# RobotLocomotion/pytorch-dense-correspondence

Measured on AMD Instinct MI355X. Metric: training images/sec, 640x480 D=3 ResNet34-8s, higher is better.
Workload: dtype f32 (f16x3 products)

## Files before the change

### pytorch-dense-correspondence_amd/csrc/dcn_common.h

```cpp
#pragma once
#include <hip/hip_runtime.h>
#include <stdint.h>

#include "dcn_hip.h"

#ifndef DCN_WAIT_VMCNT
#define DCN_WAIT_VMCNT(n) asm volatile("s_waitcnt vmcnt(" #n ")" ::: "memory")
#define DCN_WAIT_LGKMCNT0() asm volatile("s_waitcnt lgkmcnt(0)" ::: "memory")
#define DCN_OPAQUE_INT(v) asm volatile("" : "+v"(v))
#endif

#if defined(DCN_HOSTEMU_BUILD)
#define DCN_MAX_VGPRS(n)
#else
#define DCN_MAX_VGPRS(n) __attribute__((amdgpu_num_vgpr(n)))
#endif

#define DCN_SCHED_FENCE() do { asm volatile("" ::: "memory"); __builtin_amdgcn_sched_barrier(0); } while (0)

namespace dcn {

constexpr int kWave = 64;

template <class T> __device__ __forceinline__ T wave_sum(T v) {
#pragma unroll
    for (int off = kWave / 2; off > 0; off >>= 1) v += __shfl_down(v, off, kWave);
    return v;
}

template <int NT, class T> __device__ __forceinline__ T block_sum(T v, T* scratch) {
    v = wave_sum(v);
    const int lane = threadIdx.x & (kWave - 1), wv = threadIdx.x / kWave;
    __syncthreads();
    if (lane == 0) scratch[wv] = v;
    __syncthreads();
    T r = scratch[0];
    if (threadIdx.x == 0) {
#pragma unroll
        for (int i = 1; i < NT / kWave; ++i) r += scratch[i];
    }
    return r;
}

static __global__ void __launch_bounds__(256) fill_words_kernel(unsigned* __restrict__ p, unsigned v, size_t words) {
    for (size_t i = (size_t)blockIdx.x * 256 + threadIdx.x; i < words; i += (size_t)gridDim.x * 256) p[i] = v;
}
inline int fill_bytes_async(void* p, int byte_value, size_t n, hipStream_t st) {
    if (n == 0) return DCN_OK;
    if (n % 4) return DCN_E_INVALID;
    const unsigned b = (unsigned)byte_value & 0xffu, v = b | (b << 8) | (b << 16) | (b << 24);
    const size_t words = n / 4;
    size_t blocks = (words + 255) / 256;
    if (blocks > 4096) blocks = 4096;
    hipLaunchKernelGGL(fill_words_kernel, dim3((unsigned)blocks), dim3(256), 0, st, (unsigned*)p, v, words);
    return hipGetLastError() == hipSuccess ? DCN_OK : DCN_E_LAUNCH;
}

inline int check_launch() { return hipGetLastError() == hipSuccess ? DCN_OK : DCN_E_LAUNCH; }

__host__ __device__ inline int64_t ceil_div64(int64_t a, int64_t b) { return (a + b - 1) / b; }
__host__ __device__ inline int ceil_div(int a, int b) { return (a + b - 1) / b; }

}
```

### pytorch-dense-correspondence_amd/csrc/dcn_tuning.h

```cpp
#pragma once

namespace dcn {

struct Tuning {
    int conv_mode = -1;
    int conv_mode_invalid = 0;
    int backward_overlap = 1;
    int gemm_tile_m = 0;
    int gemm_sk = -1;
    double gemm_sk_min_gain = 20.0;
    int gemm_uni = 1;
    int stem8 = 1;
    int gemm_sk_inline = 1;
    int bn_bwd_fused = 0;
    int defer_residual_add = 1;
    int wgrad_splits = 0;
    int wgrad_tile = 0;
    int wgrad_deep = 4;
    int gemm_hl = 1;
    int hl_min_k = 128;
    int gemm_hl_rows = 0;
    int gemm_hlx = 1;
    int gemm_hlx_kg = 0;
    int gemm_hlx_splits = 0;
    int gemm_hlx_narrow = 1;
    double hlx_cost1 = 1.32, hlx_cost2 = 1.42, hlx_split_cost = 14.0;
    int hl_setprio = 1;
    int hlx_stagger = 1;
    int hlx_counters = 1;
    int wgrad_hl_min_m = 0;
    int wgrad_hl = 1;
    int wgrad_hlr = 1;
    int wgrad_hlr_min_m = 0;
    int wgrad_hlr_pairs = 1;
    int hl_producers = 1;
    int hl_only_mid = 1;
    int stem_pool_fused = 1;
    int bn_reduce_wide = 32;
    int wsplit_overlap = 1;
    int bn_nt = 0;
    int bn_reverse = 0;
    int bn_bwd_lean = 1;
    int bn_bwd_lean_mask = 7;
    int wgrad_roles = 1;
};

const Tuning& tuning();

}
```

### pytorch-dense-correspondence_amd/csrc/dcn_tuning.hip

```cpp
#include <atomic>
#include <cstdio>
#include <cstdlib>
#include <cstring>
#include <mutex>

#include "dcn_common.h"
#include "dcn_tuning.h"

namespace dcn {
namespace {

Tuning g_tuning;
std::once_flag g_once;
std::mutex g_mu;

void read_env(Tuning& t) {
    t = Tuning();
    if (const char* m = getenv("DCN_CONV_MODE")) {
        if (!strcmp(m, "fp32")) t.conv_mode = DCN_CONV_FP32;
        else if (!strcmp(m, "f16x3")) t.conv_mode = DCN_CONV_F16X3;
        else t.conv_mode_invalid = 1;
    }
    if (const char* e = getenv("DCN_BACKWARD_OVERLAP")) t.backward_overlap = atoi(e) != 0;
    if (const char* e = getenv("DCN_GEMM_TILE_M")) t.gemm_tile_m = atoi(e);
    if (const char* e = getenv("DCN_GEMM_SK")) t.gemm_sk = atoi(e);
    if (const char* e = getenv("DCN_GEMM_SK_MIN_GAIN")) t.gemm_sk_min_gain = atof(e);
    if (const char* e = getenv("DCN_STEM8")) t.stem8 = atoi(e) != 0;
    if (const char* e = getenv("DCN_GEMM_UNI")) t.gemm_uni = atoi(e) != 0;
    if (const char* e = getenv("DCN_GEMM_SK_FIXUP")) t.gemm_sk_inline = strcmp(e, "kernel") != 0;
    if (const char* e = getenv("DCN_BN_BWD_FUSED")) t.bn_bwd_fused = atoi(e) != 0;
    if (const char* e = getenv("DCN_DEFER_RESIDUAL_ADD")) t.defer_residual_add = atoi(e) != 0;
    if (const char* e = getenv("DCN_WGRAD_DEEP")) t.wgrad_deep = atoi(e);
    if (const char* e = getenv("DCN_WGRAD_ROLES")) t.wgrad_roles = atoi(e);
    if (const char* e = getenv("DCN_WGRAD_TILE")) t.wgrad_tile = atoi(e);
    if (const char* e = getenv("DCN_WGRAD_SPLITS")) t.wgrad_splits = atoi(e);
    if (const char* e = getenv("DCN_GEMM_HL")) t.gemm_hl = atoi(e);
    if (const char* e = getenv("DCN_GEMM_HL_ROWS")) t.gemm_hl_rows = atoi(e);
    if (const char* e = getenv("DCN_HL_MIN_K")) { const int v = atoi(e); if (v >= 32) t.hl_min_k = v; }
    if (const char* e = getenv("DCN_GEMM_HLX")) {
        int a = 0, b = 0;
        if (strchr(e, ',')) {
            if (sscanf(e, "%d,%d", &a, &b) == 2) {
                t.gemm_hlx = 1;
                t.gemm_hlx_kg = (a == 1 || a == 2) ? a : 0;
                t.gemm_hlx_splits = b > 0 ? b : 0;
            }
        } else {
            t.gemm_hlx = atoi(e) != 0;
        }
    }
    if (const char* e = getenv("DCN_GEMM_HLX_NARROW")) t.gemm_hlx_narrow = atoi(e) != 0;
    if (const char* e = getenv("DCN_HLX_COST")) {
        double a = 0, b = 0, c = 0;
        if (sscanf(e, "%lf,%lf,%lf", &a, &b, &c) == 3 && a > 0 && b > 0 && c >= 0) { t.hlx_cost1 = a; t.hlx_cost2 = b; t.hlx_split_cost = c; }
    }
    if (const char* e = getenv("DCN_HL_ONLY_MID")) t.hl_only_mid = atoi(e);
    if (const char* e = getenv("DCN_STEM_POOL_FUSED")) t.stem_pool_fused = atoi(e);
    if (const char* e = getenv("DCN_WGRAD_HL")) t.wgrad_hl = atoi(e);
    if (const char* e = getenv("DCN_HL_SETPRIO")) t.hl_setprio = atoi(e) != 0;
    if (const char* e = getenv("DCN_HLX_STAGGER")) { const int v = atoi(e); t.hlx_stagger = (v >= 0 && v <= 2) ? v : 1; }
    if (const char* e = getenv("DCN_HLX_COUNTERS")) t.hlx_counters = atoi(e) != 0;
    if (const char* e = getenv("DCN_WGRAD_HL_MIN_M")) t.wgrad_hl_min_m = atoi(e);
    if (const char* e = getenv("DCN_WGRAD_HLR")) t.wgrad_hlr = atoi(e);
    if (const char* e = getenv("DCN_WGRAD_HLR_MIN_M")) t.wgrad_hlr_min_m = atoi(e);
    if (const char* e = getenv("DCN_WGRAD_HLR_PAIRS")) t.wgrad_hlr_pairs = atoi(e);
    if (const char* e = getenv("DCN_HL_PRODUCERS")) t.hl_producers = atoi(e) != 0;
    if (const char* e = getenv("DCN_BN_REVERSE")) t.bn_reverse = atoi(e);
    if (const char* e = getenv("DCN_BN_NT")) t.bn_nt = atoi(e);
    if (const char* e = getenv("DCN_WSPLIT_OVERLAP")) t.wsplit_overlap = atoi(e) != 0;
    if (const char* e = getenv("DCN_BN_REDUCE_WIDE")) t.bn_reduce_wide = atoi(e);
    if (const char* e = getenv("DCN_BN_BWD_LEAN")) t.bn_bwd_lean = atoi(e) != 0;
    if (const char* e = getenv("DCN_BN_BWD_LEAN_MASK")) t.bn_bwd_lean_mask = atoi(e) & 7;
}

}

const Tuning& tuning() {
    std::call_once(g_once, [] { read_env(g_tuning); });
    return g_tuning;
}

}

extern "C" void dcn_reload_env(void) {
    (void)dcn::tuning();
    std::lock_guard<std::mutex> lock(dcn::g_mu);
    dcn::read_env(dcn::g_tuning);
}
```

### pytorch-dense-correspondence_amd/csrc/elementwise_kernels.hip

```cpp
#include "dcn_tuning.h"
#include "elementwise_kernels.h"
#include "f16_split.h"

namespace dcn {

__device__ __forceinline__ void wave_atomic_absmax(float amax, float* absmax) {
#pragma unroll
    for (int o = 32; o > 0; o >>= 1) amax = fmaxf(amax, __shfl_xor(amax, o));
    if ((threadIdx.x & 63) == 0 && amax > 0.f) {
        const unsigned bits = __float_as_uint(amax);
        if (bits > __atomic_load_n(reinterpret_cast<unsigned*>(absmax), __ATOMIC_RELAXED))
            atomicMax(reinterpret_cast<unsigned*>(absmax), bits);
    }
}

__global__ void __launch_bounds__(256)
nchw3_to_nhwc4_kernel(const float* __restrict__ img, float* __restrict__ out, int hw, int64_t total,
                      float* __restrict__ absmax) {
    __shared__ float s_m[4];
    float m = 0.f;
    for (int64_t i = (int64_t)blockIdx.x * 256 + threadIdx.x; i < total; i += (int64_t)gridDim.x * 256) {
        const int64_t n = i / hw, p = i - n * hw;
        const float* s = img + n * 3 * hw + p;
        const float4 v = make_float4(s[0], s[hw], s[2 * (int64_t)hw], 0.f);
// ... 411 lines not shown
        dgamma[c] = (float)tot_b;
    }
    if (absmax && threadIdx.x < 64) {
        bound = fmaxf(bound, __shfl_xor(bound, 1));
        bound = fmaxf(bound, __shfl_xor(bound, 2));
        if (threadIdx.x == 0) {
            const unsigned bits = __float_as_uint(bound);
            const unsigned seen = LEAN ? __atomic_load_n(reinterpret_cast<unsigned*>(absmax), __ATOMIC_RELAXED) : pre_bound;
            if (bound > 0.f && bits > seen)
                atomicMax(reinterpret_cast<unsigned*>(absmax), bits);
        }
    }
}
#define DCN_BN_FIN_ARGS const float* __restrict__ partial, int chunks, int groups, int C, double count,                        \
                        const float* __restrict__ gamma, const float* __restrict__ invstd, int gstride,                        \
                        float* __restrict__ dgamma, float* __restrict__ dbeta, float* __restrict__ k123, float* __restrict__ absmax
#define DCN_BN_FIN_PASS partial, chunks, groups, C, count, gamma, invstd, gstride, dgamma, dbeta, k123, absmax
__global__ void __launch_bounds__(256)
bn_bwd_finalize_kernel(DCN_BN_FIN_ARGS) { bn_bwd_finalize_body<false>(DCN_BN_FIN_PASS); }
__global__ void __launch_bounds__(256) DCN_MAX_VGPRS(48)
bn_bwd_finalize_lean_kernel(DCN_BN_FIN_ARGS) { bn_bwd_finalize_body<true>(DCN_BN_FIN_PASS); }
#undef DCN_BN_FIN_ARGS
#undef DCN_BN_FIN_PASS

__global__ void __launch_bounds__(256)
bn_bwd_apply_kernel(const float* __restrict__ dy, const float* dy2, const float* __restrict__ relu_out,
                    const unsigned char* __restrict__ relu_mask, const float* __restrict__ x,
                    const float* __restrict__ mean, const float* __restrict__ invstd, const float* __restrict__ k1,
                    const float* __restrict__ k2, const float* __restrict__ k3, float* __restrict__ dx,
                    float* g_out, int c4n, int64_t total4, int64_t group4, int gstride, int kstride, int rev) {
    for (int64_t j = (int64_t)blockIdx.x * 256 + threadIdx.x; j < total4; j += (int64_t)gridDim.x * 256) {
        const int64_t i = rev ? total4 - 1 - j : j;
        const int c0 = (int)(i % c4n) * 4;
        const bool second = i >= group4;
        const int c = c0 + (second ? gstride : 0), ck = c0 + (second ? kstride : 0);
        const float4 g = relu_masked(load_dy(dy, dy2, i), relu_out, relu_mask, i);
        const float4 v = reinterpret_cast<const float4*>(x)[i];
        const float4 mu = *reinterpret_cast<const float4*>(mean + c);
        const float4 is = *reinterpret_cast<const float4*>(invstd + c);
        const float4 a = *reinterpret_cast<const float4*>(k1 + ck);
        const float4 b = *reinterpret_cast<const float4*>(k2 + ck);
        const float4 d = *reinterpret_cast<const float4*>(k3 + ck);
        float4 o;
        o.x = a.x * (g.x - b.x - (v.x - mu.x) * is.x * d.x);
        o.y = a.y * (g.y - b.y - (v.y - mu.y) * is.y * d.y);
        o.z = a.z * (g.z - b.z - (v.z - mu.z) * is.z * d.z);
        o.w = a.w * (g.w - b.w - (v.w - mu.w) * is.w * d.w);
        reinterpret_cast<float4*>(dx)[i] = o;
        if (g_out) reinterpret_cast<float4*>(g_out)[i] = g;
    }
}

template <bool LEAN, bool DQ>
__device__ __forceinline__ void
bn_bwd_apply_blocked_body(const float* __restrict__ dy, const float* dy2, const float* __restrict__ relu_out,
                          const unsigned char* __restrict__ relu_mask, const float* __restrict__ x,
                          const float* __restrict__ mean, const float* __restrict__ invstd, const float* __restrict__ k1,
                          const float* __restrict__ k2, const float* __restrict__ k3, float* __restrict__ dx,
                          float* g_out, dcnsplit::u32x4* __restrict__ dq, const float* __restrict__ absmax,
                          int c4n, int64_t rows, int64_t rows_per_group, int gstride, int kstride,
                          dcnsplit::u32x2* __restrict__ hl, int rev, int nt) {
    const float s = dcnsplit::pow2_scale(*absmax);
    const int64_t total = ((rows + 3) >> 2) * c4n;
    for (int64_t j = (int64_t)blockIdx.x * 256 + threadIdx.x; j < total; j += (int64_t)gridDim.x * 256) {
        const int64_t i = rev ? total - 1 - j : j;
        const int64_t q = i / c4n;
        const int cq = (int)(i - q * c4n);
        const bool second = q * 4 >= rows_per_group;
        int c = cq * 4 + (second ? gstride : 0), ck = cq * 4 + (second ? kstride : 0);
        float4 mu, is, a, b, d;
        if (!LEAN) {
            mu = *reinterpret_cast<const float4*>(mean + c);
            is = *reinterpret_cast<const float4*>(invstd + c);
            a = *reinterpret_cast<const float4*>(k1 + ck);
            b = *reinterpret_cast<const float4*>(k2 + ck);
            d = *reinterpret_cast<const float4*>(k3 + ck);
        }
        float o[4][4];
#pragma unroll
        for (int r = 0; r < 4; ++r) {
            const int64_t m = q * 4 + r;
            if (LEAN) __builtin_amdgcn_sched_barrier(0);
            if (m < rows) {
                const int64_t e = m * c4n + cq;

                float4 g0 = ld4(dy, e, nt != 0);
                if (dy2) {
                    const float4 h = reinterpret_cast<const float4*>(dy2)[e];
                    g0.x += h.x; g0.y += h.y; g0.z += h.z; g0.w += h.w;
                }
                float4 g = relu_masked(g0, relu_out, relu_mask, e);
                float4 v = ld4(x, e, nt != 0);
                if (LEAN) {
                    DCN_OPAQUE_INT(g.x); DCN_OPAQUE_INT(g.y); DCN_OPAQUE_INT(g.z); DCN_OPAQUE_INT(g.w);
                    DCN_OPAQUE_INT(v.x); DCN_OPAQUE_INT(v.y); DCN_OPAQUE_INT(v.z); DCN_OPAQUE_INT(v.w);
                    DCN_OPAQUE_INT(c); DCN_OPAQUE_INT(ck);
                }
                if (LEAN && DQ) {
#define DCN_BN_STEP(dst, expr, ptr)                                                                                           \
                    { const float4 k = *reinterpret_cast<const float4*>(ptr);                                                  \
                      dst = expr;                                                                                              \
                      DCN_OPAQUE_INT(dst.x); DCN_OPAQUE_INT(dst.y); DCN_OPAQUE_INT(dst.z); DCN_OPAQUE_INT(dst.w); }
                    float4 t, u;
                    DCN_BN_STEP(t, make_float4(v.x - k.x, v.y - k.y, v.z - k.z, v.w - k.w), mean + c)
                    DCN_BN_STEP(t, make_float4(t.x * k.x, t.y * k.y, t.z * k.z, t.w * k.w), invstd + c)
                    DCN_BN_STEP(t, make_float4(t.x * k.x, t.y * k.y, t.z * k.z, t.w * k.w), k3 + ck)
                    DCN_BN_STEP(u, make_float4(g.x - k.x, g.y - k.y, g.z - k.z, g.w - k.w), k2 + ck)
                    DCN_BN_STEP(t, make_float4(k.x * (u.x - t.x), k.y * (u.y - t.y), k.z * (u.z - t.z), k.w * (u.w - t.w)), k1 + ck)
#undef DCN_BN_STEP
                    o[r][0] = t.x; o[r][1] = t.y; o[r][2] = t.z; o[r][3] = t.w;
                } else {
                    if (LEAN) {
                        mu = *reinterpret_cast<const float4*>(mean + c);
                        is = *reinterpret_cast<const float4*>(invstd + c);
                        a = *reinterpret_cast<const float4*>(k1 + ck);
                        b = *reinterpret_cast<const float4*>(k2 + ck);
                        d = *reinterpret_cast<const float4*>(k3 + ck);
                    }
                    o[r][0] = a.x * (g.x - b.x - (v.x - mu.x) * is.x * d.x);
                    o[r][1] = a.y * (g.y - b.y - (v.y - mu.y) * is.y * d.y);
                    o[r][2] = a.z * (g.z - b.z - (v.z - mu.z) * is.z * d.z);
                    o[r][3] = a.w * (g.w - b.w - (v.w - mu.w) * is.w * d.w);
                }
                if (dx) reinterpret_cast<float4*>(dx)[e] = make_float4(o[r][0], o[r][1], o[r][2], o[r][3]);
                if (g_out) reinterpret_cast<float4*>(g_out)[e] = g;
                if (hl) {
                    dcnsplit::h4 ha, hb;
                    dcnsplit::split4(make_float4(o[r][0], o[r][1], o[r][2], o[r][3]), s, ha, hb);
                    dcnsplit::u32x2* line = hl + (e >> 3) * 16 + (e & 7);
                    line[0] = __builtin_bit_cast(dcnsplit::u32x2, ha);
                    line[8] = __builtin_bit_cast(dcnsplit::u32x2, hb);
                }
            } else {
                o[r][0] = o[r][1] = o[r][2] = o[r][3] = 0.f;
            }
        }
        if (DQ && dq) dcnsplit::store_blocked_quad(dq, q, cq, c4n, o, s);
    }
}
#define DCN_BN_APB_ARGS const float* __restrict__ dy, const float* dy2, const float* __restrict__ relu_out,                    \
                        const unsigned char* __restrict__ relu_mask, const float* __restrict__ x,                              \
                        const float* __restrict__ mean, const float* __restrict__ invstd, const float* __restrict__ k1,        \
                        const float* __restrict__ k2, const float* __restrict__ k3, float* __restrict__ dx,                    \
                        float* g_out, dcnsplit::u32x4* __restrict__ dq, const float* __restrict__ absmax,                      \
                        int c4n, int64_t rows, int64_t rows_per_group, int gstride, int kstride,                               \
                        dcnsplit::u32x2* __restrict__ hl, int rev, int nt
#define DCN_BN_APB_PASS dy, dy2, relu_out, relu_mask, x, mean, invstd, k1, k2, k3, dx, g_out, dq, absmax, c4n, rows, rows_per_group, \
                        gstride, kstride, hl, rev, nt
__global__ void __launch_bounds__(256)
bn_bwd_apply_blocked_kernel(DCN_BN_APB_ARGS) { bn_bwd_apply_blocked_body<false, true>(DCN_BN_APB_PASS); }
template <bool DQ>
__global__ void __launch_bounds__(256) DCN_MAX_VGPRS(48)
bn_bwd_apply_blocked_lean_kernel(DCN_BN_APB_ARGS) { bn_bwd_apply_blocked_body<true, DQ>(DCN_BN_APB_PASS); }
#undef DCN_BN_APB_ARGS
#undef DCN_BN_APB_PASS

__global__ void __launch_bounds__(256)
absmax_kernel(const float* __restrict__ v, int64_t total, float* __restrict__ absmax) {
    float amax = 0.f;
    for (int64_t i = (int64_t)blockIdx.x * 256 + threadIdx.x; i < total; i += (int64_t)gridDim.x * 256)
        amax = fmaxf(amax, fabsf(v[i]));
    wave_atomic_absmax(amax, absmax);
}

__global__ void __launch_bounds__(256)
add_kernel(const float* __restrict__ a, const float* __restrict__ b, float* __restrict__ out, int64_t total4) {
    for (int64_t i = (int64_t)blockIdx.x * 256 + threadIdx.x; i < total4; i += (int64_t)gridDim.x * 256) {
        const float4 u = reinterpret_cast<const float4*>(a)[i], v = reinterpret_cast<const float4*>(b)[i];
        reinterpret_cast<float4*>(out)[i] = make_float4(u.x + v.x, u.y + v.y, u.z + v.z, u.w + v.w);
    }
}

__global__ void __launch_bounds__(256)
maxpool_fwd_kernel(const float* __restrict__ in, float* __restrict__ out, unsigned char* __restrict__ argmax, int hin,
                   int win, int hout, int wout, int c4n, int64_t total4, const float* __restrict__ scale,
                   const float* __restrict__ shift, int gstride, int64_t group_n, unsigned char* __restrict__ relu_mask) {
    const int64_t i = (int64_t)blockIdx.x * 256 + threadIdx.x;
    if (i >= total4) return;
    const int c4 = (int)(i % c4n);
    int64_t pix = i / c4n;
    const int ox = (int)(pix % wout); pix /= wout;
    const int oy = (int)(pix % hout);
    const int64_t n = pix / hout;
    float4 sc = make_float4(1.f, 1.f, 1.f, 1.f), sh = make_float4(0.f, 0.f, 0.f, 0.f);
    if (scale) {
        const int c = c4 * 4 + (n >= group_n ? gstride : 0);
        sc = *reinterpret_cast<const float4*>(scale + c);
        sh = *reinterpret_cast<const float4*>(shift + c);
    }
    float4 best = make_float4(-INFINITY, -INFINITY, -INFINITY, -INFINITY);
    int bx = -1, by = -1, bz = -1, bw = -1;
    for (int r = 0; r < 3; ++r) {
        const int iy = oy * 2 - 1 + r;
        if (iy < 0 || iy >= hin) continue;
        for (int s = 0; s < 3; ++s) {
            const int ix = ox * 2 - 1 + s;
            if (ix < 0 || ix >= win) continue;
            const int64_t src = ((n * hin + iy) * win + ix) * c4n + c4;
            float4 v = reinterpret_cast<const float4*>(in)[src];
            if (scale) {
                v = make_float4(v.x * sc.x + sh.x, v.y * sc.y + sh.y, v.z * sc.z + sh.z, v.w * sc.w + sh.w);
                v.x = fmaxf(v.x, 0.f); v.y = fmaxf(v.y, 0.f); v.z = fmaxf(v.z, 0.f); v.w = fmaxf(v.w, 0.f);
                if (relu_mask)
                    relu_mask[src] = (unsigned char)((v.x > 0.f ? 1 : 0) | (v.y > 0.f ? 2 : 0) | (v.z > 0.f ? 4 : 0) | (v.w > 0.f ? 8 : 0));
            }
            const int t = r * 3 + s;
            if (v.x > best.x || bx < 0 || v.x != v.x) { best.x = v.x; bx = t; }
            if (v.y > best.y || by < 0 || v.y != v.y) { best.y = v.y; by = t; }
            if (v.z > best.z || bz < 0 || v.z != v.z) { best.z = v.z; bz = t; }
            if (v.w > best.w || bw < 0 || v.w != v.w) { best.w = v.w; bw = t; }
        }
    }
    reinterpret_cast<float4*>(out)[i] = best;
    if (argmax) {
        unsigned char* a = argmax + i * 4;
        a[0] = (unsigned char)bx; a[1] = (unsigned char)by; a[2] = (unsigned char)bz; a[3] = (unsigned char)bw;
    }
}

__global__ void __launch_bounds__(256)
maxpool_bwd_kernel(const float* __restrict__ gout, const float* __restrict__ gout2, const unsigned char* __restrict__ argmax,
                   float* __restrict__ gin, int hin, int win, int hout, int wout, int c4n, int64_t total4) {
    const int64_t i = (int64_t)blockIdx.x * 256 + threadIdx.x;
    if (i >= total4) return;
    const int c4 = (int)(i % c4n);
    int64_t pix = i / c4n;
    const int ix = (int)(pix % win); pix /= win;
    const int iy = (int)(pix % hin);
    const int64_t n = pix / hin;
    float4 acc = make_float4(0.f, 0.f, 0.f, 0.f);
    for (int oy = iy / 2; oy <= (iy + 1) / 2; ++oy) {
        if (oy >= hout) continue;
        const int r = iy - (oy * 2 - 1);
        if (r < 0 || r > 2) continue;
        for (int ox = ix / 2; ox <= (ix + 1) / 2; ++ox) {
            if (ox >= wout) continue;
            const int s = ix - (ox * 2 - 1);
            if (s < 0 || s > 2) continue;
            const int t = r * 3 + s;
            const int64_t o = ((n * hout + oy) * wout + ox) * c4n + c4;
            float4 g = reinterpret_cast<const float4*>(gout)[o];
            if (gout2) {
                const float4 h = reinterpret_cast<const float4*>(gout2)[o];
                g.x += h.x; g.y += h.y; g.z += h.z; g.w += h.w;
            }
            const unsigned char* a = argmax + o * 4;
            if (a[0] == t) acc.x += g.x;
            if (a[1] == t) acc.y += g.y;
            if (a[2] == t) acc.z += g.z;
            if (a[3] == t) acc.w += g.w;
        }
    }
    reinterpret_cast<float4*>(gin)[i] = acc;
}

__device__ __forceinline__ void src_index(int dst, float scale, int in_size, int& i0, int& i1, float& l1) {
    const float s = scale * (float)dst;
    i0 = (int)s;
    if (i0 > in_size - 1) i0 = in_size - 1;
    i1 = i0 < in_size - 1 ? i0 + 1 : i0;
    l1 = s - (float)i0;
}

__global__ void __launch_bounds__(256)
upsample_fwd_kernel(const float* __restrict__ low, int hl, int wl, int ldl, int d, int h, int w, float sh, float sw,
                    int normalize, float* __restrict__ out, int64_t total) {
    const int64_t i = (int64_t)blockIdx.x * 256 + threadIdx.x;
    if (i >= total) return;
    const int x = (int)(i % w);
    const int64_t t = i / w;
    const int y = (int)(t % h);
    const int64_t n = t / h;
    int y0, y1, x0, x1;
    float ly, lx;
    src_index(y, sh, hl, y0, y1, ly);
    src_index(x, sw, wl, x0, x1, lx);
    const float hy = 1.f - ly, hx = 1.f - lx;
    const float* p00 = low + ((n * hl + y0) * wl + x0) * ldl;
    const float* p01 = low + ((n * hl + y0) * wl + x1) * ldl;
    const float* p10 = low + ((n * hl + y1) * wl + x0) * ldl;
    const float* p11 = low + ((n * hl + y1) * wl + x1) * ldl;
    float* o = out + i * d;
    if (!normalize) {
        for (int k = 0; k < d; ++k) o[k] = hy * (hx * p00[k] + lx * p01[k]) + ly * (hx * p10[k] + lx * p11[k]);
    } else {
        float ss = 0.f;
        for (int k = 0; k < d; ++k) {
            const float v = hy * (hx * p00[k] + lx * p01[k]) + ly * (hx * p10[k] + lx * p11[k]);
            ss = fmaf(v, v, ss);
        }
        const float nrm = sqrtf(ss);
        for (int k = 0; k < d; ++k)
            o[k] = (hy * (hx * p00[k] + lx * p01[k]) + ly * (hx * p10[k] + lx * p11[k])) / nrm;
    }
}

__global__ void __launch_bounds__(256)
normalize_bwd_kernel(const float* __restrict__ low, int hl, int wl, int ldl, int d, int h, int w, float sh, float sw,
                     const float* __restrict__ gout, float* __restrict__ gv, int64_t total) {
    const int64_t i = (int64_t)blockIdx.x * 256 + threadIdx.x;
    if (i >= total) return;
    const int x = (int)(i % w);
    const int64_t t = i / w;
    const int y = (int)(t % h);
    const int64_t n = t / h;
    int y0, y1, x0, x1;
    float ly, lx;
    src_index(y, sh, hl, y0, y1, ly);
    src_index(x, sw, wl, x0, x1, lx);
    const float hy = 1.f - ly, hx = 1.f - lx;
    const float* p00 = low + ((n * hl + y0) * wl + x0) * ldl;
    const float* p01 = low + ((n * hl + y0) * wl + x1) * ldl;
    const float* p10 = low + ((n * hl + y1) * wl + x0) * ldl;
    const float* p11 = low + ((n * hl + y1) * wl + x1) * ldl;
    const float* g = gout + i * d;
    float ss = 0.f, dot = 0.f;
    for (int k = 0; k < d; ++k) {
        const float v = hy * (hx * p00[k] + lx * p01[k]) + ly * (hx * p10[k] + lx * p11[k]);
        ss = fmaf(v, v, ss);
        dot = fmaf(v, g[k], dot);
    }
    const float nrm = sqrtf(ss), inv = 1.f / nrm;
    dot *= inv;
    for (int k = 0; k < d; ++k) {
        const float v = hy * (hx * p00[k] + lx * p01[k]) + ly * (hx * p10[k] + lx * p11[k]);
        gv[i * d + k] = (g[k] - v * inv * dot) * inv;
    }
}

__global__ void __launch_bounds__(256)
upsample_bwd_rows_kernel(const float* __restrict__ gout, int hl, int d, int h, int w, float sh, float* __restrict__ tmp,
                         int64_t total) {
    const int64_t i = (int64_t)blockIdx.x * 256 + threadIdx.x;
    if (i >= total) return;
    const int64_t wd = (int64_t)w * d;
    const int64_t xd = i % wd;
    const int64_t t = i / wd;
    const int iy = (int)(t % hl);
    const int64_t n = t / hl;
    const float inv = sh > 0.f ? 1.f / sh : 0.f;
    int ylo = (int)floorf(((float)iy - 1.f) * inv) - 1, yhi = (int)ceilf(((float)iy + 1.f) * inv) + 1;
    if (ylo < 0) ylo = 0;
    if (yhi > h - 1 || sh <= 0.f) yhi = h - 1;
    float acc = 0.f;
    for (int y = ylo; y <= yhi; ++y) {
        int y0, y1;
        float ly;
        src_index(y, sh, hl, y0, y1, ly);
        float wgt = 0.f;
        if (y0 == iy) wgt += 1.f - ly;
        if (y1 == iy) wgt += ly;
        if (wgt != 0.f) acc = fmaf(wgt, gout[(n * h + y) * wd + xd], acc);
    }
    tmp[i] = acc;
}
__global__ void __launch_bounds__(256)
upsample_bwd_cols_kernel(const float* __restrict__ tmp, int hl, int wl, int ldl, int d, int w, float sw,
                         float* __restrict__ glow, int64_t total) {
    const int64_t i = (int64_t)blockIdx.x * 256 + threadIdx.x;
    if (i >= total) return;
    const int k = (int)(i % ldl);
    const int64_t t = i / ldl;
    const int ix = (int)(t % wl);
    const int64_t row = t / wl;
    if (k >= d) { glow[i] = 0.f; return; }
    const float inv = sw > 0.f ? 1.f / sw : 0.f;
    int xlo = (int)floorf(((float)ix - 1.f) * inv) - 1, xhi = (int)ceilf(((float)ix + 1.f) * inv) + 1;
    if (xlo < 0) xlo = 0;
    if (xhi > w - 1 || sw <= 0.f) xhi = w - 1;
    float acc = 0.f;
    for (int x = xlo; x <= xhi; ++x) {
        int x0, x1;
        float lx;
        src_index(x, sw, wl, x0, x1, lx);
        float wgt = 0.f;
        if (x0 == ix) wgt += 1.f - lx;
        if (x1 == ix) wgt += lx;
        if (wgt != 0.f) acc = fmaf(wgt, tmp[(row * w + x) * d + k], acc);
    }
    glow[i] = acc;
}

static inline unsigned blocks_for(int64_t n, int cap = 0) {
    int64_t b = ceil_div64(n, 256);
    if (cap > 0 && b > cap) b = cap;
    if (b < 1) b = 1;
    return (unsigned)b;
}
constexpr int kGridCap = 256 * 8;

thread_local const LaunchObserver* launch_observer = nullptr;

void launch_nchw3_to_nhwc4(const float* img, float* out, int n, int hw, float* absmax, hipStream_t st) {
    const int64_t total = (int64_t)n * hw;
    ObservedLaunch obs(DCN_PROF_RESAMPLE, 28.0 * (double)total, st);
    hipLaunchKernelGGL(nchw3_to_nhwc4_kernel, dim3(blocks_for(total, kGridCap)), dim3(256), 0, st, img, out, hw, total, absmax);
}
void launch_pad_c3_to_c4(const float* w, float* wp, int64_t rows, hipStream_t st) {
    ObservedLaunch obs(DCN_PROF_OTHER, 28.0 * (double)rows, st);
    hipLaunchKernelGGL(pad_c3_to_c4_kernel, dim3(blocks_for(rows)), dim3(256), 0, st, w, wp, rows);
}
void launch_unpad_c4_to_c3(const float* wp, float* w, int64_t rows, hipStream_t st) {
    ObservedLaunch obs(DCN_PROF_OTHER, 28.0 * (double)rows, st);
    hipLaunchKernelGGL(unpad_c4_to_c3_kernel, dim3(blocks_for(rows)), dim3(256), 0, st, wp, w, rows);
}
void launch_pad_rows(const float* src, float* dst, int64_t rows, int d, int ld, hipStream_t st) {
    ObservedLaunch obs(DCN_PROF_OTHER, 4.0 * (double)rows * (d + ld), st);
    hipLaunchKernelGGL(pad_rows_kernel, dim3(blocks_for(rows * ld)), dim3(256), 0, st, src, dst, rows, d, ld);
}
void launch_bn_finalize(const float* partial, int tiles_per_group, int groups, int C, double count_per_group,
                        const float* gamma, const float* beta, float* rmean, float* rvar, float momentum, float eps,
                        int training, float* stats, float* out_bound, const float* res_bound, hipStream_t st) {
    ObservedLaunch obs(DCN_PROF_BN_FINALIZE, training ? 12.0 * (double)tiles_per_group * groups * C : 0.0, st);
    hipLaunchKernelGGL(bn_finalize_kernel, dim3(ceil_div(C, 4)), dim3(256), 0, st, partial, tiles_per_group, groups, C,
                       count_per_group, gamma, beta, rmean, rvar, momentum, eps, training, stats, stats + C, stats + 2 * C,
                       stats + 3 * C, 4 * C, out_bound, res_bound);
}
void launch_bn_apply(const float* x, const float* stats1, const float* res, const float* stats2, int relu, float* y,
                     unsigned char* relu_mask, int C, int64_t rows, int groups, hipStream_t st, void* hl_out,
                     const float* hl_absmax) {
    const int64_t total4 = rows * (C / 4);
    if ((C % 32) != 0 || !hl_absmax) hl_out = nullptr;
    ObservedLaunch obs(DCN_PROF_BN_APPLY, (double)rows * C * (4.0 + (res ? 4.0 : 0.0) + (y ? 4.0 : 0.0) + (hl_out ? 4.0 : 0.0) +
                                                             (relu_mask ? 0.25 : 0.0)), st);
    hipLaunchKernelGGL(bn_apply_kernel, dim3(blocks_for(total4, kGridCap)), dim3(256), 0, st, x, stats1, stats1 + C, res,
                       stats2, stats2 ? stats2 + C : nullptr, relu, y, relu_mask, C / 4, total4, total4 / groups, 4 * C,
                       (dcnsplit::u32x2*)hl_out, hl_absmax, tuning().bn_reverse & 1, tuning().bn_nt & 1);
}
int bn_bwd_chunks(int64_t rows_per_group) {
    const int rows = rows_per_group >= 16384 ? 128 : (rows_per_group >= 8192 ? 64 : 32);
    int64_t chunks = ceil_div64(rows_per_group, rows);
    if (chunks > 1024) chunks = 1024;
    if (chunks < 1) chunks = 1;
    return (int)chunks;
}
void launch_bn_bwd(const float* dy, const float* relu_out, const unsigned char* relu_mask, const float* x, const float* stats,
                   const float* gamma, int C,
                   int64_t rows, int groups, float* partial, float* dgamma, float* dbeta, float* k123, float* dx,
                   float* g_out, float* absmax, void* dq, hipStream_t st, int reduced_tiles_per_group, const float* dy2,
                   void* hl_dx, int keep_dx, int lean) {
    const int64_t rpg = rows / groups;
    const float* mean = stats + 2 * C;
    const float* invstd = stats + 3 * C;
    int chunks = reduced_tiles_per_group;
    const double in_bytes = 8.0 + (dy2 ? 4.0 : 0.0) + (relu_mask ? 0.25 : (relu_out ? 4.0 : 0.0));
    if (chunks <= 0) {
        chunks = bn_bwd_chunks(rpg);
        const int rpc = (int)ceil_div64(rpg, chunks);
        ObservedLaunch obs(DCN_PROF_BN_BWD_REDUCE, (double)rows * C * in_bytes, st);
        const int cap = tuning().bn_reduce_wide;
        const int cq = ((C % 512) == 0 && cap >= 128) ? 128 : (((C % 256) == 0 && cap >= 64) ? 64 : (((C % 128) == 0 && cap >= 32) ? 32 : 16));
#define DCN_BN_RED(K, CQ)                                                                                                     \
        hipLaunchKernelGGL(K<CQ>, dim3(ceil_div(C, 4 * CQ), chunks * groups), dim3(256), 0, st, dy, dy2, relu_out,            \
                           relu_mask, x, mean, invstd, C, rpg, chunks, 4 * C, rpc, partial)
#define DCN_BN_RED_CQ(K)                                                                                                      \
        if (cq == 128) DCN_BN_RED(K, 128);                                                                                    \
        else if (cq == 64) DCN_BN_RED(K, 64);                                                                                 \
        else if (cq == 32) DCN_BN_RED(K, 32);                                                                                 \
        else DCN_BN_RED(K, 16)
        if (lean & 1) { DCN_BN_RED_CQ(bn_bwd_reduce_lean_kernel); }
        else { DCN_BN_RED_CQ(bn_bwd_reduce_kernel); }
#undef DCN_BN_RED_CQ
#undef DCN_BN_RED
    }
    {
        ObservedLaunch obs(DCN_PROF_BN_FINALIZE, 16.0 * (double)chunks * groups * C, st);
        const auto kernel = (lean & 2) ? bn_bwd_finalize_lean_kernel : bn_bwd_finalize_kernel;
        hipLaunchKernelGGL(kernel, dim3(ceil_div(C, 4)), dim3(256), 0, st,
                           (const float*)partial, chunks, groups, C, (double)rpg, gamma, invstd, 4 * C, dgamma, dbeta, k123, absmax);
    }
    const int64_t total4 = rows * (C / 4);
    if ((dq || (hl_dx && (C % 32) == 0)) && absmax) {
        const bool hl = hl_dx && (C % 32) == 0;
        ObservedLaunch obs(DCN_PROF_BN_BWD_APPLY, (double)rows * C * (in_bytes + ((hl && !keep_dx) ? 0.0 : 4.0) + (g_out ? 4.0 : 0.0) +
                                                                      (dq ? 4.0 : 0.0) + (hl ? 4.0 : 0.0)), st);
        const auto kernel = !(lean & 4) ? bn_bwd_apply_blocked_kernel
                                        : (dq ? bn_bwd_apply_blocked_lean_kernel<true> : bn_bwd_apply_blocked_lean_kernel<false>);
        hipLaunchKernelGGL(kernel, dim3(blocks_for(((rows + 3) / 4) * (C / 4), kGridCap)), dim3(256), 0, st,
                           dy, dy2, relu_out, relu_mask, x, mean, invstd, (const float*)k123, (const float*)(k123 + C),
                           (const float*)(k123 + 2 * C), (hl_dx && (C % 32) == 0 && !keep_dx) ? nullptr : dx, g_out,
                           (dcnsplit::u32x4*)dq, (const float*)absmax, C / 4, rows, rpg, 4 * C, 3 * C,
                           (C % 32) == 0 ? (dcnsplit::u32x2*)hl_dx : nullptr, (tuning().bn_reverse >> 1) & 1, (tuning().bn_nt >> 1) & 1);
        return;
    }
    ObservedLaunch obs(DCN_PROF_BN_BWD_APPLY, (double)rows * C * (in_bytes + 4.0 + (g_out ? 4.0 : 0.0)), st);
    hipLaunchKernelGGL(bn_bwd_apply_kernel, dim3(blocks_for(total4, kGridCap)), dim3(256), 0, st, dy, dy2, relu_out, relu_mask,
                       x, mean, invstd, (const float*)k123, (const float*)(k123 + C), (const float*)(k123 + 2 * C), dx, g_out,
                       C / 4, total4, total4 / groups, 4 * C, 3 * C, (tuning().bn_reverse >> 1) & 1);
}
void launch_add(const float* a, const float* b, float* out, int64_t n, hipStream_t st) {
    ObservedLaunch obs(DCN_PROF_OTHER, 12.0 * (double)n, st);
    hipLaunchKernelGGL(add_kernel, dim3(blocks_for(n / 4, kGridCap)), dim3(256), 0, st, a, b, out, n / 4);
}
void launch_maxpool_fwd(const float* in, float* out, unsigned char* argmax, int n, int hin, int win, int hout,
                        int wout, int C, hipStream_t st, const float* bn_stats, int groups, unsigned char* relu_mask) {
    const int64_t total4 = (int64_t)n * hout * wout * (C / 4);
    ObservedLaunch obs(DCN_PROF_RESAMPLE, (double)n * C * ((double)hin * win * (4.0 + (bn_stats && relu_mask ? 0.25 : 0.0)) +
                                                          (double)hout * wout * (4.0 + (argmax ? 1.0 : 0.0))), st);
    hipLaunchKernelGGL(maxpool_fwd_kernel, dim3(blocks_for(total4)), dim3(256), 0, st, in, out, argmax, hin, win, hout,
                       wout, C / 4, total4, bn_stats, bn_stats ? bn_stats + C : nullptr, 4 * C,
                       (int64_t)(groups > 1 ? n / groups : n), bn_stats ? relu_mask : nullptr);
}
void launch_maxpool_bwd(const float* gout, const unsigned char* argmax, float* gin, int n, int hin, int win, int hout,
                        int wout, int C, hipStream_t st, const float* gout2) {
    const int64_t total4 = (int64_t)n * hin * win * (C / 4);
    ObservedLaunch obs(DCN_PROF_RESAMPLE, (double)n * C * ((double)hin * win * 4.0 + (double)hout * wout * (5.0 + (gout2 ? 4.0 : 0.0))), st);
    hipLaunchKernelGGL(maxpool_bwd_kernel, dim3(blocks_for(total4)), dim3(256), 0, st, gout, gout2, argmax, gin, hin, win,
                       hout, wout, C / 4, total4);
}
static inline float ac_scale(int in, int out) { return out > 1 ? (float)(in - 1) / (float)(out - 1) : 0.f; }
void launch_upsample_fwd(const float* low, int n, int hl, int wl, int ldl, int d, int h, int w, int normalize,
                         float* out, hipStream_t st) {
    const int64_t total = (int64_t)n * h * w;
    ObservedLaunch obs(DCN_PROF_RESAMPLE, 4.0 * ((double)n * hl * wl * ldl + (double)total * d), st);
    hipLaunchKernelGGL(upsample_fwd_kernel, dim3(blocks_for(total)), dim3(256), 0, st, low, hl, wl, ldl, d, h, w,
                       ac_scale(hl, h), ac_scale(wl, w), normalize, out, total);
}
size_t upsample_bwd_tmp_bytes(int n, int hl, int w, int d) { return (size_t)n * hl * w * d * sizeof(float); }
void launch_normalize_bwd(const float* low, int n, int hl, int wl, int ldl, int d, int h, int w, const float* gout,
                          float* gv, hipStream_t st) {
    const int64_t total = (int64_t)n * h * w;
    ObservedLaunch obs(DCN_PROF_RESAMPLE, 4.0 * ((double)n * hl * wl * ldl + 2.0 * (double)total * d), st);
    hipLaunchKernelGGL(normalize_bwd_kernel, dim3(blocks_for(total)), dim3(256), 0, st, low, hl, wl, ldl, d, h, w,
                       ac_scale(hl, h), ac_scale(wl, w), gout, gv, total);
}
void launch_upsample_bwd(const float* gout, int n, int hl, int wl, int ldl, int d, int h, int w, float* tmp,
                         float* glow, float* absmax, hipStream_t st, const float* gout_b) {
    const int64_t t1 = (int64_t)n * hl * w * d;
    if (gout_b) {
        const int64_t th = t1 / 2;
        for (int k = 0; k < 2; ++k) {
            ObservedLaunch obs(DCN_PROF_RESAMPLE, 4.0 * ((double)(n / 2) * h * w * d + (double)th), st);
            hipLaunchKernelGGL(upsample_bwd_rows_kernel, dim3(blocks_for(th)), dim3(256), 0, st, k ? gout_b : gout, hl, d, h, w,
                               ac_scale(hl, h), tmp + k * th, th);
        }
    } else {
        ObservedLaunch obs(DCN_PROF_RESAMPLE, 4.0 * ((double)n * h * w * d + (double)t1), st);
        hipLaunchKernelGGL(upsample_bwd_rows_kernel, dim3(blocks_for(t1)), dim3(256), 0, st, gout, hl, d, h, w,
                           ac_scale(hl, h), tmp, t1);
    }
    const int64_t t2 = (int64_t)n * hl * wl * ldl;
    {
        ObservedLaunch obs(DCN_PROF_RESAMPLE, 4.0 * ((double)t1 + (double)t2), st);
        hipLaunchKernelGGL(upsample_bwd_cols_kernel, dim3(blocks_for(t2)), dim3(256), 0, st, (const float*)tmp, hl, wl, ldl,
                           d, w, ac_scale(wl, w), glow, t2);
    }
    if (absmax) {
        ObservedLaunch obs(DCN_PROF_OTHER, 4.0 * (double)t2, st);
        hipLaunchKernelGGL(absmax_kernel, dim3(blocks_for(t2, 256)), dim3(256), 0, st, (const float*)glow, t2, absmax);
    }
}

}

extern "C" int dcn_upsample_forward(const float* low, int n, int hl, int wl, int ldl, int d, int h, int w, int normalize,
                                    float* out, void* stream) {
    if (!low || !out || n < 1 || hl < 1 || wl < 1 || d < 1 || ldl < d || h < 1 || w < 1) return DCN_E_INVALID;
    dcn::launch_upsample_fwd(low, n, hl, wl, ldl, d, h, w, normalize, out, (hipStream_t)stream);
    return dcn::check_launch();
}

extern "C" size_t dcn_upsample_backward_tmp_bytes(int n, int hl, int w, int d) {
    return dcn::upsample_bwd_tmp_bytes(n, hl, w, d);
}

extern "C" int dcn_upsample_backward(const float* gout, int n, int hl, int wl, int ldl, int d, int h, int w, float* glow,
                                     float* tmp, void* stream) {
    if (!gout || !glow || !tmp || n < 1 || hl < 1 || wl < 1 || d < 1 || ldl < d || h < 1 || w < 1) return DCN_E_INVALID;
    dcn::launch_upsample_bwd(gout, n, hl, wl, ldl, d, h, w, tmp, glow, nullptr, (hipStream_t)stream);
    return dcn::check_launch();
}

extern "C" int dcn_bn_forward(const float* x, const float* bn_partial, int mtiles, int c, int64_t rows, const float* gamma,
                              const float* beta, float* running_mean, float* running_var, float momentum, float eps,
                              int training, const float* res, int relu, float* y, unsigned char* relu_mask, float* stats,
                              void* stream) {
    if (!x || !gamma || !beta || !y || !stats || c < 4 || (c % 4) != 0 || rows < 1) return DCN_E_INVALID;
    if (training ? (!bn_partial || mtiles < 1) : (!running_mean || !running_var)) return DCN_E_INVALID;
    hipStream_t st = (hipStream_t)stream;
    dcn::launch_bn_finalize(bn_partial, mtiles, 1, c, (double)rows, gamma, beta, running_mean, running_var, momentum, eps,
                            training, stats, nullptr, nullptr, st);
    dcn::launch_bn_apply(x, stats, res, nullptr, relu, y, relu_mask, c, rows, 1, st);
    return dcn::check_launch();
}

extern "C" size_t dcn_bn_backward_workspace(int64_t rows, int c) {
    if (rows < 1 || c < 4) return 0;
    return ((size_t)dcn::bn_bwd_chunks(rows) * 4 * (size_t)c + 3 * (size_t)c) * sizeof(float);
}

extern "C" int dcn_bn_backward(const float* dy, const unsigned char* relu_mask, const float* x, const float* stats,
                               const float* gamma, int c, int64_t rows, float* dgamma, float* dbeta, float* dx, float* g_out,
                               void* workspace, void* stream) {
    if (!dy || !x || !stats || !gamma || !dgamma || !dbeta || !dx || !workspace || c < 4 || (c % 4) != 0 || rows < 1)
        return DCN_E_INVALID;
    float* partial = (float*)workspace;
    float* k123 = partial + (size_t)dcn::bn_bwd_chunks(rows) * 4 * c;
    dcn::launch_bn_bwd(dy, nullptr, relu_mask, x, stats, gamma, c, rows, 1, partial, dgamma, dbeta, k123, dx, g_out, nullptr,
                       nullptr, (hipStream_t)stream, 0, nullptr, nullptr, 0, dcn::tuning().bn_bwd_lean ? dcn::tuning().bn_bwd_lean_mask : 0);
    return dcn::check_launch();
}

extern "C" int dcn_bn_backward_from_partial(const float* dy, const float* bn_partial, int mtiles, const float* x,
                                            const float* stats, const float* gamma, int c, int64_t rows, float* dgamma,
                                            float* dbeta, float* dx, void* workspace, void* stream) {
    if (!dy || !bn_partial || mtiles < 1 || !x || !stats || !gamma || !dgamma || !dbeta || !dx || !workspace || c < 4 ||
        (c % 4) != 0 || rows < 1)
        return DCN_E_INVALID;
    dcn::launch_bn_bwd(dy, nullptr, nullptr, x, stats, gamma, c, rows, 1, const_cast<float*>(bn_partial), dgamma, dbeta,
                       (float*)workspace, dx, nullptr, nullptr, nullptr, (hipStream_t)stream, mtiles, nullptr, nullptr, 0,
                       dcn::tuning().bn_bwd_lean ? dcn::tuning().bn_bwd_lean_mask : 0);
    return dcn::check_launch();
}

extern "C" size_t dcn_bn_backward_full_workspace(int64_t rows, int c, int groups) {
    if (rows < 1 || c < 4 || groups < 1 || (rows % groups) != 0) return 0;
    return ((size_t)groups * dcn::bn_bwd_chunks(rows / groups) * 4 * (size_t)c + (size_t)groups * 3 * (size_t)c) * sizeof(float);
}

extern "C" int dcn_bn_backward_full(const float* dy, const float* dy2, const float* relu_out, const unsigned char* relu_mask,
                                    const float* x, const float* stats, const float* gamma, int c, int64_t rows, int groups,
                                    float* dgamma, float* dbeta, float* dx, float* g_out, float* absmax, void* dq, void* hl_dx,
                                    int keep_dx, void* workspace, void* stream) {
    if (!dy || !x || !stats || !gamma || !dgamma || !dbeta || !workspace || c < 4 || (c % 4) != 0 || rows < 1) return DCN_E_INVALID;
    if ((groups != 1 && groups != 2) || (rows % groups) != 0) return DCN_E_INVALID;
    const bool blocked = (dq || (hl_dx && (c % 32) == 0)) && absmax;
    if ((dq || hl_dx) && !absmax) return DCN_E_INVALID;
    if (hl_dx && (c % 32) != 0) return DCN_E_INVALID;
    if (blocked && groups == 2 && ((rows / groups) % 4) != 0) return DCN_E_INVALID;
    if (!dx && !(hl_dx && !keep_dx)) return DCN_E_INVALID;
// ... 21 lines not shown
```

Baseline: 470.0.

## Add software-pipelined deep BN backward apply kernel with LDS-staged coefficients

Adds a new blocked BN backward apply kernel that issues loads for several rows ahead (depth 2 or 3) before computing, so memory latency overlaps with arithmetic. Per-channel mean, invstd and k coefficients are staged once per block in shared memory instead of being reloaded per element. Specialised template variants remove runtime branches for the mask, dy2, dx, g_out and hl outputs. It is selected by default for C<=512 and up to two groups. The cost is more register pressure under a 48-VGPR cap and more code variants.

Result: faster. 481.7 (median of 6 runs) (+2.5%).

```diff
diff --git a/pytorch-dense-correspondence_amd/csrc/dcn_common.h b/pytorch-dense-correspondence_amd/csrc/dcn_common.h
--- a/pytorch-dense-correspondence_amd/csrc/dcn_common.h
+++ b/pytorch-dense-correspondence_amd/csrc/dcn_common.h
@@ -14,6 +14,12 @@
 #define DCN_MAX_VGPRS(n)
 #else
 #define DCN_MAX_VGPRS(n) __attribute__((amdgpu_num_vgpr(n)))
+#endif
+
+#if defined(DCN_HOSTEMU_BUILD)
+#define DCN_OPAQUE_UNIFORM(v) ((void)(v))
+#else
+#define DCN_OPAQUE_UNIFORM(v) asm volatile("" : "+s"(v))
 #endif
 
 #define DCN_SCHED_FENCE() do { asm volatile("" ::: "memory"); __builtin_amdgcn_sched_barrier(0); } while (0)
diff --git a/pytorch-dense-correspondence_amd/csrc/dcn_tuning.h b/pytorch-dense-correspondence_amd/csrc/dcn_tuning.h
--- a/pytorch-dense-correspondence_amd/csrc/dcn_tuning.h
+++ b/pytorch-dense-correspondence_amd/csrc/dcn_tuning.h
@@ -42,6 +42,7 @@
     int bn_reverse = 0;
     int bn_bwd_lean = 1;
     int bn_bwd_lean_mask = 7;
+    int bn_bwd_lean_depth = 3;
     int wgrad_roles = 1;
 };
 
diff --git a/pytorch-dense-correspondence_amd/csrc/dcn_tuning.hip b/pytorch-dense-correspondence_amd/csrc/dcn_tuning.hip
--- a/pytorch-dense-correspondence_amd/csrc/dcn_tuning.hip
+++ b/pytorch-dense-correspondence_amd/csrc/dcn_tuning.hip
@@ -71,6 +71,7 @@
     if (const char* e = getenv("DCN_BN_REDUCE_WIDE")) t.bn_reduce_wide = atoi(e);
     if (const char* e = getenv("DCN_BN_BWD_LEAN")) t.bn_bwd_lean = atoi(e) != 0;
     if (const char* e = getenv("DCN_BN_BWD_LEAN_MASK")) t.bn_bwd_lean_mask = atoi(e) & 7;
+    if (const char* e = getenv("DCN_BN_BWD_LEAN_DEPTH")) { const int v = atoi(e); t.bn_bwd_lean_depth = v < 1 ? 1 : (v > 3 ? 3 : v); }
 }
 
 }
diff --git a/pytorch-dense-correspondence_amd/csrc/elementwise_kernels.hip b/pytorch-dense-correspondence_amd/csrc/elementwise_kernels.hip
--- a/pytorch-dense-correspondence_amd/csrc/elementwise_kernels.hip
+++ b/pytorch-dense-correspondence_amd/csrc/elementwise_kernels.hip
@@ -587,6 +587,145 @@
 template <bool DQ>
 __global__ void __launch_bounds__(256) DCN_MAX_VGPRS(48)
 bn_bwd_apply_blocked_lean_kernel(DCN_BN_APB_ARGS) { bn_bwd_apply_blocked_body<true, DQ>(DCN_BN_APB_PASS); }
+
+struct BnBwdRow { float4 g, h, v; unsigned m; };
+__device__ __forceinline__ const float* bn_at(const float* p, unsigned bytes) {
+    return reinterpret_cast<const float*>(reinterpret_cast<const char*>(p) + bytes);
+}
+template <bool DY2, bool MASK>
+__device__ __forceinline__ void bn_bwd_row_issue(BnBwdRow& w, const float* x_b, const float* dy_b, const float* dy2_b,
+                                                 const unsigned char* mask_b, unsigned o) {
+    w.v = *reinterpret_cast<const float4*>(bn_at(x_b, 16u * o));
+    w.g = *reinterpret_cast<const float4*>(bn_at(dy_b, 16u * o));
+    if (DY2) w.h = *reinterpret_cast<const float4*>(bn_at(dy2_b, 16u * o));
+    if (MASK) w.m = mask_b[o];
+}
+template <bool DY2, bool MASK>
+__device__ __forceinline__ float4 bn_bwd_row_grad(const BnBwdRow& w) {
+    float4 g = w.g;
+    if (DY2) { g.x += w.h.x; g.y += w.h.y; g.z += w.h.z; g.w += w.h.w; }
+    if (MASK) {
+        const unsigned m = w.m;
+        g.x = (m & 1u) ? g.x : 0.f; g.y = (m & 2u) ? g.y : 0.f; g.z = (m & 4u) ? g.z : 0.f; g.w = (m & 8u) ? g.w : 0.f;
+    }
+    return g;
+}
+#define DCN_OPAQUE_F4(v) do { DCN_OPAQUE_INT(v.x); DCN_OPAQUE_INT(v.y); DCN_OPAQUE_INT(v.z); DCN_OPAQUE_INT(v.w); } while (0)
+constexpr int kBnDeepPitch = 2 * 128;
+template <int D, bool DQ, bool DY2, bool MASK, int GOUT, int DX, int HL, bool GUARD>
+__device__ __forceinline__ void
+bn_bwd_apply_deep_body(int64_t j0, const float* __restrict__ dy, const float* dy2, const unsigned char* __restrict__ relu_mask,
+                       const float* __restrict__ x, float* __restrict__ dx, float* g_out, dcnsplit::u32x4* __restrict__ dq,
+                       float s, int c4n, int64_t rows, int64_t rows_per_group, dcnsplit::u32x2* __restrict__ hl, const float4* s_k) {
+    DCN_OPAQUE_UNIFORM(c4n);
+    const unsigned uc4n = (unsigned)c4n;
+    const int64_t q0 = j0 / c4n;
+    const int64_t eb = q0 * 4 * c4n;
+    const int64_t left = rows - q0 * 4, gleft = rows_per_group - q0 * 4, live_n = ((rows + 3) >> 2) * c4n - q0 * c4n;
+    const unsigned nrow = left < (1 << 20) ? (unsigned)left : (1u << 20);
+    const unsigned grow = gleft <= 0 ? 0u : (gleft < (1 << 20) ? (unsigned)gleft : (1u << 20));
+    const unsigned nlive = live_n < (1 << 20) ? (unsigned)live_n : (1u << 20);
+    const unsigned lim = nrow * uc4n - 1u;
+    const float* x_b = x + eb * 4;
+    const float* dy_b = dy + eb * 4;
+    const float* dy2_b = DY2 ? dy2 + eb * 4 : dy2;
+    const unsigned char* mask_b = MASK ? relu_mask + eb : relu_mask;
+    const unsigned rel = (unsigned)(j0 - q0 * c4n) + threadIdx.x;
+    const unsigned qr = rel / uc4n, cq = rel - qr * uc4n;
+    unsigned er = qr * 4u * uc4n + cq;
+    unsigned sec = qr * 4u >= grow ? 1u : 0u;
+    DCN_OPAQUE_INT(sec);
+    unsigned ks = (sec << 7) + cq;
+    unsigned row0 = qr * 4u, rows_l = rel < nlive ? nrow : 0u;
+    DCN_OPAQUE_INT(er); DCN_OPAQUE_INT(ks);
+    if (GUARD) { DCN_OPAQUE_INT(row0); DCN_OPAQUE_INT(rows_l); }
+    const float4* kp = s_k + ks;
+    BnBwdRow w[4];
+    float o[4][4];
+    auto issue = [&](int r) {
+        const unsigned e = er + (unsigned)r * uc4n;
+        bn_bwd_row_issue<DY2, MASK>(w[r], x_b, dy_b, dy2_b, mask_b, GUARD ? (e < lim ? e : lim) : e);
+    };
+#pragma unroll
+    for (int r = 0; r < D; ++r) issue(r);
+    DCN_SCHED_FENCE();
+#pragma unroll
+    for (int r = 0; r < 4; ++r) {
+        float4 g = bn_bwd_row_grad<DY2, MASK>(w[r]);
+        float4 t = w[r].v, u, k;
+        DCN_OPAQUE_F4(g); DCN_OPAQUE_F4(t);
+        k = kp[0];                 t = make_float4(t.x - k.x, t.y - k.y, t.z - k.z, t.w - k.w); DCN_OPAQUE_F4(t); DCN_SCHED_FENCE();
+        k = kp[kBnDeepPitch];      t = make_float4(t.x * k.x, t.y * k.y, t.z * k.z, t.w * k.w); DCN_OPAQUE_F4(t); DCN_SCHED_FENCE();
+        k = kp[2 * kBnDeepPitch];  t = make_float4(t.x * k.x, t.y * k.y, t.z * k.z, t.w * k.w); DCN_OPAQUE_F4(t); DCN_SCHED_FENCE();
+        k = kp[3 * kBnDeepPitch];  u = make_float4(g.x - k.x, g.y - k.y, g.z - k.z, g.w - k.w); DCN_OPAQUE_F4(u); DCN_SCHED_FENCE();
+        k = kp[4 * kBnDeepPitch];
+        t = make_float4(k.x * (u.x - t.x), k.y * (u.y - t.y), k.z * (u.z - t.z), k.w * (u.w - t.w)); DCN_OPAQUE_F4(t);
+        const bool in = !GUARD || row0 + (unsigned)r < rows_l;
+        if (DQ) {
+            o[r][0] = in ? t.x : 0.f; o[r][1] = in ? t.y : 0.f; o[r][2] = in ? t.z : 0.f; o[r][3] = in ? t.w : 0.f;
+        }
+        if (in) {
+            unsigned e = er;
+            DCN_OPAQUE_INT(e);
+            e += (unsigned)r * uc4n;
+            if (DX == 1 || (DX == 2 && dx)) *reinterpret_cast<float4*>(const_cast<float*>(bn_at(dx + eb * 4, 16u * e))) = t;
+            if (GOUT == 1 || (GOUT == 2 && g_out)) *reinterpret_cast<float4*>(const_cast<float*>(bn_at(g_out + eb * 4, 16u * e))) = g;
+            if (HL == 1 || (HL == 2 && hl)) {
+                __builtin_amdgcn_sched_barrier(0);
+                dcnsplit::h2 a0, b0, a1, b1;
+                dcnsplit::split2(t.x * s, t.y * s, a0, b0);
+                __builtin_amdgcn_sched_barrier(0);
+                dcnsplit::split2(t.z * s, t.w * s, a1, b1);
+                const dcnsplit::h4 ha = {a0[0], a0[1], a1[0], a1[1]}, hb = {b0[0], b0[1], b1[0], b1[1]};
+                dcnsplit::u32x2* line = reinterpret_cast<dcnsplit::u32x2*>(reinterpret_cast<char*>(hl + (eb >> 3) * 16) +
+                                                                             8u * ((e >> 3) * 16u + (e & 7u)));
+                line[0] = __builtin_bit_cast(dcnsplit::u32x2, ha);
+                line[8] = __builtin_bit_cast(dcnsplit::u32x2, hb);
+            }
+        }
+        if (DQ) { DCN_OPAQUE_INT(o[r][0]); DCN_OPAQUE_INT(o[r][1]); DCN_OPAQUE_INT(o[r][2]); DCN_OPAQUE_INT(o[r][3]); }
+        DCN_SCHED_FENCE();
+        if (r + D < 4) { issue(r + D); DCN_SCHED_FENCE(); }
+    }
+    if (DQ && dq && (!GUARD || row0 < rows_l))
+        dcnsplit::store_blocked_quad(reinterpret_cast<dcnsplit::u32x4*>(reinterpret_cast<char*>(dq + eb) + 16u * er), 0, 0, c4n, o, s);
+}
+template <int D, bool DQ>
+__global__ void __launch_bounds__(256) DCN_MAX_VGPRS(48)
+bn_bwd_apply_blocked_deep_kernel(DCN_BN_APB_ARGS) {
+    __shared__ float4 s_k[5 * kBnDeepPitch];
+    const int ng = rows_per_group < rows ? 2 : 1;
+    for (int i = threadIdx.x; i < ng * 5 * c4n; i += 256) {
+        const int g = i / (5 * c4n), n = (i - g * 5 * c4n) / c4n, cq = i - (g * 5 + n) * c4n;
+        const float* src = n == 0 ? mean + g * gstride : (n == 1 ? invstd + g * gstride : ((n == 2 ? k3 : (n == 3 ? k2 : k1)) + g * kstride));
+        s_k[n * kBnDeepPitch + g * 128 + cq] = *reinterpret_cast<const float4*>(src + 4 * cq);
+    }
+    __syncthreads();
+    const float s = __builtin_bit_cast(float, __builtin_amdgcn_readfirstlane(__builtin_bit_cast(int, dcnsplit::pow2_scale(*absmax))));
+    const int64_t total = ((rows + 3) >> 2) * c4n;
+    for (int64_t j0 = (int64_t)blockIdx.x * 256; j0 < total; j0 += (int64_t)gridDim.x * 256) {
+        const bool whole = j0 + 256 <= total && ((j0 + 255) / c4n) * 4 + 3 < rows;
+#define DCN_BN_DEEP(DD, DY2, MASK, GOUT, DX, HL, GUARD)                                                                        \
+        bn_bwd_apply_deep_body<DD, DQ, DY2, MASK, GOUT, DX, HL, GUARD>(j0, dy, dy2, relu_mask, x, dx, g_out, dq, s, c4n, rows,  \
+                                                                       rows_per_group, hl, s_k)
+#define DCN_BN_DEEP_DX(DD, DY2, MASK, HL)                                                                                      \
+        do {                                                                                                                   \
+            if (g_out) { if (dx) DCN_BN_DEEP(DD, DY2, MASK, 1, 1, HL, false); else DCN_BN_DEEP(DD, DY2, MASK, 1, 0, HL, false); } \
+            else { if (dx) DCN_BN_DEEP(DD, DY2, MASK, 0, 1, HL, false); else DCN_BN_DEEP(DD, DY2, MASK, 0, 0, HL, false); }     \
+        } while (0)
+#define DCN_BN_DEEP_OUT(DD, DY2, MASK)                                                                                         \
+        do {                                                                                                                   \
+            if (!whole) DCN_BN_DEEP(((DQ && DY2) ? 1 : DD), DY2, MASK, 2, 2, 2, true);                                                            \
+            else if (DQ && !hl) DCN_BN_DEEP_DX(DD, DY2, MASK, 0);                                                              \
+            else DCN_BN_DEEP_DX(DD, DY2, MASK, 1);                                                                             \
+        } while (0)
+        if (relu_mask) { if (dy2) DCN_BN_DEEP_OUT(2, true, true); else DCN_BN_DEEP_OUT(D, false, true); }
+        else { if (dy2) DCN_BN_DEEP_OUT(2, true, false); else DCN_BN_DEEP_OUT(D, false, false); }
+#undef DCN_BN_DEEP_OUT
+#undef DCN_BN_DEEP_DX
+#undef DCN_BN_DEEP
+    }
+}
 #undef DCN_BN_APB_ARGS
 #undef DCN_BN_APB_PASS
 
@@ -878,6 +1017,8 @@
     const float* mean = stats + 2 * C;
     const float* invstd = stats + 3 * C;
     int chunks = reduced_tiles_per_group;
+    const int depth = tuning().bn_bwd_lean_depth;
+    const bool deep = depth > 1 && !(relu_out && !relu_mask);
     const double in_bytes = 8.0 + (dy2 ? 4.0 : 0.0) + (relu_mask ? 0.25 : (relu_out ? 4.0 : 0.0));
     if (chunks <= 0) {
         chunks = bn_bwd_chunks(rpg);
@@ -909,8 +1050,11 @@
         const bool hl = hl_dx && (C % 32) == 0;
         ObservedLaunch obs(DCN_PROF_BN_BWD_APPLY, (double)rows * C * (in_bytes + ((hl && !keep_dx) ? 0.0 : 4.0) + (g_out ? 4.0 : 0.0) +
                                                                       (dq ? 4.0 : 0.0) + (hl ? 4.0 : 0.0)), st);
+        const bool deep_apply = deep && C <= 512 && groups <= 2;
         const auto kernel = !(lean & 4) ? bn_bwd_apply_blocked_kernel
-                                        : (dq ? bn_bwd_apply_blocked_lean_kernel<true> : bn_bwd_apply_blocked_lean_kernel<false>);
+                            : (!deep_apply ? (dq ? bn_bwd_apply_blocked_lean_kernel<true> : bn_bwd_apply_blocked_lean_kernel<false>)
+                               : (dq ? bn_bwd_apply_blocked_deep_kernel<2, true>
+                                     : (depth > 2 ? bn_bwd_apply_blocked_deep_kernel<3, false> : bn_bwd_apply_blocked_deep_kernel<2, false>)));
         hipLaunchKernelGGL(kernel, dim3(blocks_for(((rows + 3) / 4) * (C / 4), kGridCap)), dim3(256), 0, st,
                            dy, dy2, relu_out, relu_mask, x, mean, invstd, (const float*)k123, (const float*)(k123 + C),
                            (const float*)(k123 + 2 * C), (hl_dx && (C % 32) == 0 && !keep_dx) ? nullptr : dx, g_out,
```
